# jizongFox/Contrast-You

Hardware: AMD Instinct MI355X
Metric: 2D slices/sec on ACDC U-Net+InfoNCE step (higher is better)
Workload: dtype bf16; 1 GPU; C2: ACDC SemiSupervisedEpocher + InfoNCE@Conv5 (partition), two-stage, 16 labeled + 16 unlabeled 1x224x224 per GPU, 4 classes, UNet max_channel=512, RAdam; global_batch=32, parallelism=dp1

## Files before the change

### contrast-you_amd/contrastyou/arch/unet.py

```python
from __future__ import annotations

from collections import OrderedDict
from contextlib import contextmanager
from enum import Enum
from functools import partial
from typing import Optional

import torch
from torch import Tensor, nn

from cyhip import ops
from cyhip.functions import (ChainCfg, ConvChainFn, HeadFn, begin_pass, compute_dtype_for, defer_batch_counters,
                             prepack)

from ._base import _check_params, _complete_arch_start2end
from .utils import get_bn_track, get_requires_grad

__all__ = ["UNet", "UNetFeatureMapEnum"]


def _conv3x3(cin: int, cout: int) -> nn.Conv2d:
    return nn.Conv2d(cin, cout, kernel_size=(3, 3), stride=(1, 1), padding=(1, 1), bias=False)


# ... 93 lines not shown
        self._Up_conv2 = _ConvBlock(ch("Up_conv3"), ch("Up_conv2"), momentum)

        self._Deconv_1x1 = _Head1x1(ch("Up_conv2"), num_classes, kernel_size=(1, 1), stride=(1, 1),
                                    padding=(0, 0))
        self._compute_dtype: Optional[torch.dtype] = None
        for tag, names in (("decoder", self.decoder_names), ("conv5", ("Conv5",)), ("conv4", ("Conv4",))):
            for n in names:
                for p in getattr(self, f"_{n}").parameters():
                    p.__dict__["_cy_ready_tag"] = tag
        self._Up5.ready_tag, self._Conv5.ready_tag, self._Conv4.ready_tag = "decoder", "conv5", "conv4"

    @property
    def compute_dtype(self) -> Optional[torch.dtype]:
        return self._compute_dtype

    @compute_dtype.setter
    def compute_dtype(self, dt: Optional[torch.dtype]):
        self._compute_dtype = dt
        for m in self.modules():
            if isinstance(m, (_ConvBlock, _UpConv)):
                m.compute_dtype = dt

    def forward(self, x: Tensor, until: str = None):
        if until and until not in self.layer_dimension:
            raise KeyError(f"`return_until` should be in {', '.join(self.layer_dimension.keys())},"
                           f" given {until}  ")
        ops.require_gpu(x)
        ops.note_home_stream(x.device)
        if x.dim() != 4 or x.shape[1] != self._input_dim:
            raise ValueError(f"expected [N,{self._input_dim},H,W], got {tuple(x.shape)}")
        if x.shape[2] % 16 or x.shape[3] % 16:
            raise ValueError("spatial dims must be multiples of 16 (four 2x2 poolings)")
        begin_pass()
        prepack(self._packed_conv_weights(), compute_dtype_for(x, self._compute_dtype))
        with defer_batch_counters(x.device):
            return self._forward(x, until)

    def _packed_conv_weights(self):
        ws = []
        for m in self.modules():
            if isinstance(m, _ConvBlock):
                ws += [m.conv[3].weight] if m._first else [m.conv[0].weight, m.conv[3].weight]
            elif isinstance(m, _UpConv):
                ws.append(m.up[1].weight)
        return [w for w in ws if w.is_cuda and w.dtype == torch.float32 and w.is_contiguous()]

    def _forward(self, x: Tensor, until: Optional[str]):
        e1 = self._Conv1(x, pool_out=until != "Conv1")
        if until == "Conv1":
            return e1
        e2 = self._Conv2(self._Conv1.take_pooled(), pool_out=until != "Conv2")
        if until == "Conv2":
            return e2
        e3 = self._Conv3(self._Conv2.take_pooled(), pool_out=until != "Conv3")
        if until == "Conv3":
            return e3
        e4 = self._Conv4(self._Conv3.take_pooled(), pool_out=until != "Conv4")
        if until == "Conv4":
            return e4
        e5 = self._Conv5(self._Conv4.take_pooled())
        if until == "Conv5":
            return e5

        d5 = self._Up_conv5(e4, self._Up5(e5))
        if until == "Up_conv5":
            return d5
        d4 = self._Up_conv4(e3, self._Up4(d5))
# ... 81 lines not shown
```

### contrast-you_amd/csrc/cy_conv3x3.hip

```cpp
#include "cy_conv_plane.h"
#include "cy_conv_stream.h"
#include "cy_conv_flow.h"
#include "cy_conv_tile.h"

#include <cstdlib>

namespace {

template <typename T, typename TO, int TH, int TW, int BN, int WGM, int WGN, int PITCHB, bool ALLT>
struct ConvCfg {
  static constexpr int EPC = ElemTr<T>::EPC;
  static constexpr int KC = PITCHB / (int)sizeof(T);
  static constexpr int CPP = PITCHB / 16;
  static constexpr int KS = KC / 16;
  static constexpr int HW2 = TW + 2;
  static constexpr int ZSLOT = TH + 2;
  static constexpr int A_BYTES = (TH + 3) * HW2 * PITCHB;
  static constexpr int B_BYTES = BN * PITCHB;
  static constexpr int MT = TH * TW / 32;
  static constexpr int M_REP = MT / WGM;
  static constexpr int N_REP = BN / (32 * WGN);
  static constexpr int BREG = (BN * CPP + 255) / 256;
  static constexpr int TAB_BYTES = (3 * TH + 4) * 4;
  static constexpr int EPI_BYTES = 4 * 32 * 36 * 4 + WGM * 2 * BN * 4;
  static constexpr int NBUF = ALLT ? 9 : 2;
  static constexpr int MAIN_BYTES = A_BYTES + NBUF * B_BYTES;
  static constexpr int SMEM = (MAIN_BYTES > EPI_BYTES ? MAIN_BYTES : EPI_BYTES) + TAB_BYTES + 16;
  static_assert(WGM * WGN == 4, "4 waves");
  static_assert((TH * TW) % 32 == 0 && MT % WGM == 0, "tile/wave split");
  static_assert(BN % (32 * WGN) == 0, "cout/wave split");
  static_assert(256 % CPP == 0, "chunk ownership");
};

template <typename T, typename TO, int TH, int TW, int BN, int WGM, int WGN, int PITCHB, bool ALLT>
__global__ void __launch_bounds__(256, 2)
// ... 521 lines not shown
  TileChoice tile = choose_tile(NH, d->W, Cout);
  if (plane) tile.th = kPlaneTH, tile.tw = kPlaneTW;
  const int tiles = cy_cdiv(NH, tile.th) * cy_cdiv(d->W, tile.tw);
  if (plane) {
    tile.bn = Cout >= 128 ? 128 : (Cout > 32 ? 64 : 32);
    constexpr int bn64_below = 300;
    if (Cout == 128 && tiles < bn64_below) tile.bn = 64;
  }
  const int blocks = tiles * cy_cdiv(Cout, tile.bn);
  const int kc = (tile.bn <= 64 ? 64 : 128) / (d->in_dtype == CY_F32 ? 4 : 2);
  const int ncc = cy_cdiv(Cin, kc);
  int Z = 1;
  if (blocks < 192 && ncc >= 2 && Cout % 8 == 0) {
    Z = cy_cdiv(384, blocks);
    if (Z > ncc) Z = ncc;
    if (Z > 8) Z = 8;
  }
  bool one_per_cu = false;
  if (plane && tile.bn == 128 && ncc >= 2) {
    int z1 = blocks >= 256 ? 1 : 256 / blocks;
    if (z1 > ncc / 2) z1 = ncc / 2;
    if (z1 < 1) z1 = 1;
    if (blocks * z1 >= 192 && blocks * z1 <= 288 && Cout % 8 == 0) one_per_cu = true, Z = z1;
  }
  return make_plan(d, plane ? CY_CONV_KERNEL_PLANE : CY_CONV_KERNEL_IGEMM, tile, Z, tiles, one_per_cu);
}

ConvPlan plan_conv(const cy_conv_desc* d) {
  ConvPlan p;
  if (plan_stream(d, &p) || plan_flow(d, &p)) return p;
  return plan_tiled(d);
}

template <typename TO>
int launch_finish(const ConvArgs& a, const ConvPlan& p, hipStream_t st) {
  const int G = a.Cout / 8;
  const int gpp = G < 256 ? G : 256;
  const int rows = 256 / gpp;
  const size_t smem = (size_t)2 * rows * gpp * 8 * sizeof(float);
  hipLaunchKernelGGL(conv_splitk_finish_kernel<TO>, dim3(p.finish_blocks), dim3(256), smem, st, a.ws,
                     p.ksplit, (long)a.NH * a.W, a.Cout, (TO*)a.out, a.ldo, (TO*)a.out2, a.ldo2,
                     a.split_c, a.stats, a.sacc, a.sR);
  CY_CHECK_LAUNCH();
  return CY_OK;
}

template <typename T>
int dispatch_conv(const ConvArgs& a, const ConvPlan& p, hipStream_t st) {
  if (p.kernel == CY_CONV_KERNEL_STREAM) {
    if constexpr (sizeof(T) == 2) return dispatch_conv_stream<T>(a, st);
    return CY_ERR_DTYPE;
  }
  if (p.kernel == CY_CONV_KERNEL_FLOW) {
    if constexpr (sizeof(T) == 2) return dispatch_conv_flow<T>(a, p.tile.th, p.tile.bn, p.tile.tw, st);
    return CY_ERR_DTYPE;
  }
  if (p.kernel == CY_CONV_KERNEL_PLANE) {
    if (p.tile.bn == 128)
      return p.one_per_cu ? launch_conv_plane<T, kPlaneTH, 128, 2, 2, 128, false, true>(a, st)
                          : launch_conv_plane<T, kPlaneTH, 128, 2, 2, 128, false, false>(a, st);
    if (p.tile.bn == 64) return launch_conv_plane<T, kPlaneTH, 64, 4, 1, 64, true>(a, st);
    return launch_conv_plane<T, kPlaneTH, 32, 4, 1, 64, true>(a, st);
  }
  const TileChoice c = p.tile;
#define CY_CONV_CASE(TH_, TW_, BN_, WGM_, WGN_, P_, ALLT_) \
  return launch_conv<T, T, TH_, TW_, BN_, WGM_, WGN_, P_, ALLT_>(a, st)
// ... 589 lines not shown
  a.ksplit = p.ksplit;
  a.ws = (float*)ws;
  if (p.ksplit > 1 && (!ws || ws_bytes < p.ws_bytes)) return CY_ERR_WORKSPACE;
  hipStream_t st = (hipStream_t)stream;
  if (dz) {
    if (!dgrad_dz_plan_ok(d, p, dz->c0, dz->C)) return CY_ERR_SHAPE;
    a.dz_y = dz->y, a.dz_coef = dz->coef, a.dz_acc = (unsigned long long*)dz->acc->acc, a.dz_R = dz->acc->R;
    a.dz_ld = dz->C, a.dz_c0 = dz->c0, a.dz_C = dz->C;
  }
  if (bwd) {
    if (!dgrad_bn_plan_ok(d, p)) return CY_ERR_SHAPE;
    a.ysrc = bwd->y, a.bytes_y = a.bytes1;
    a.dy_out = bwd->dy, a.bytes_dy = a.bytes1;
    a.bfold.acc = (const unsigned long long*)bwd->acc->acc, a.bfold.R = bwd->acc->R, a.bfold.C = d->C1;
    a.bfold.coef = bwd->coef, a.bfold.inv_count = 1.0 / bwd->count, a.bfold.batch_stats = bwd->batch_stats;
    a.bfold.accumulate = bwd->accumulate, a.bfold.dgamma = bwd->dgamma, a.bfold.dbeta = bwd->dbeta;
  }
  if (in_fold) {
    if ((p.kernel == CY_CONV_KERNEL_FLOW || p.kernel == CY_CONV_KERNEL_STREAM) && cy_switches().bn_fold_in_kernel) {
      a.fold = bn_fold_from_abi(in_fold);
    } else {
      rc = cy_bn_fold_coef(in_fold, stream);
      if (rc != CY_OK) return rc;
      a.scale = in_fold->coef, a.shift = in_fold->coef + in_fold->C;
    }
  }
  rc = d->in_dtype == CY_BF16 ? dispatch_conv<bf16>(a, p, st)
       : d->in_dtype == CY_F16 ? dispatch_conv<f16>(a, p, st) : dispatch_conv<float>(a, p, st);
  if (rc != CY_OK || p.ksplit == 1) return rc;
  return d->in_dtype == CY_BF16 ? launch_finish<bf16>(a, p, st)
         : d->in_dtype == CY_F16 ? launch_finish<f16>(a, p, st) : launch_finish<float>(a, p, st);
}

int cy_debug_conv_stamps(unsigned long long* dev_buf) {
  g_conv_stamp_buf = dev_buf;
  return CY_OK;
}

int cy_conv3x3_first_num_partials(int N, int H, int W, int Cout) {
  if (Cout % 8 || Cout > 64 || 256 % (Cout / 8)) return CY_ERR_SHAPE;
  const int b = first_conv_blocks((long)N * H * W, Cout, W);
  return b < 0 ? CY_ERR_SHAPE : b;
}

static int first_fwd_impl(const float* x, const float* w, void* out, float* stats, unsigned long long* sacc, int sR, int N,
                          int Cin, int H, int W, int Cout, int out_dtype, void* stream);

int cy_conv3x3_first_fwd(const float* x, const float* w, void* out, float* stats, int N, int Cin,
                         int H, int W, int Cout, int out_dtype, void* stream) {
  return first_fwd_impl(x, w, out, stats, nullptr, 0, N, Cin, H, W, Cout, out_dtype, stream);
}

int cy_conv3x3_first_fwd_acc(const float* x, const float* w, void* out, const cy_bn_acc* out_acc, int N, int Cin,
                             int H, int W, int Cout, int out_dtype, void* stream) {
  if (!out_acc || !out_acc->acc || out_acc->C != Cout || out_acc->R < 1 || (out_acc->R & (out_acc->R - 1))) return CY_ERR_ARG;
  return first_fwd_impl(x, w, out, nullptr, (unsigned long long*)out_acc->acc, out_acc->R, N, Cin, H, W, Cout, out_dtype, stream);
}

static int first_fwd_impl(const float* x, const float* w, void* out, float* stats, unsigned long long* sacc, int sR, int N,
                          int Cin, int H, int W, int Cout, int out_dtype, void* stream) {
  if (!x || !w || !out) return CY_ERR_ARG;
  if (Cin < 1 || Cin > 4) return CY_ERR_SHAPE;
  if ((long)N * H * W >= (1L << 31)) return CY_ERR_SHAPE;
  const int np = cy_conv3x3_first_num_partials(N, H, W, Cout);
  if (np < 0) return np;
  hipStream_t st = (hipStream_t)stream;
// ... 36 lines not shown
```

### contrast-you_amd/csrc/cy_switches.h

```cpp
#pragma once
#include <cstdlib>

namespace cy_env {
static inline int as_int(const char* name, int dflt) {
  const char* e = getenv(name);
  return e ? atoi(e) : dflt;
}
static inline bool unless_0(const char* name) {
  const char* e = getenv(name);
  return !(e && e[0] == '0');
}
}

struct CySwitches {
  bool conv_plane = cy_env::unless_0("CY_CONV_PLANE");
  int stream = cy_env::as_int("CY_STREAM", 1);
  int flow = cy_env::as_int("CY_FLOW", 1);
  int flow_cfg = cy_env::as_int("CY_FLOW_CFG", 0);
  int plane_xcd = cy_env::as_int("CY_PLANE_XCD", 1);
  int dgrad_bn_all = cy_env::as_int("CY_DGRAD_BN_ALL", 0);
  int bn_fold_in_kernel = cy_env::as_int("CY_BN_FOLD_IN_KERNEL", 1);
  int first_mfma = cy_env::as_int("CY_FIRST_MFMA", 1);
  bool first_wgrad_mfma = cy_env::unless_0("CY_FIRST_WGRAD_MFMA");
  bool wgrad_spec = cy_env::unless_0("CY_WGRAD_SPEC");
  bool wgrad_dma = cy_env::unless_0("CY_WGRAD_DMA");
  bool wgrad_blk = cy_env::unless_0("CY_WGRAD_BLK");
};

__attribute__((visibility("hidden"))) inline const CySwitches& cy_switches() {
  static const CySwitches s{};
  return s;
}
```

### contrast-you_amd/cyhip/functions.py

```python
from __future__ import annotations

import contextlib
import os
from typing import List, Optional

import torch
from torch import Tensor, nn

from . import ops

_weights_epoch = 0


_nbt_pending: Optional[list] = None


_run_pending: Optional[list] = None


class defer_batch_counters:

    def __init__(self, device=None):
        self._device = device

# ... 14 lines not shown
            ops.bn_running_update(running)
            if pending:
                with ops.ordered("bn_batch_counters"):
                    torch._foreach_add_(pending, 1)
        return False


RAW_TAP = None


def bump_weights_epoch() -> None:
    global _weights_epoch
    _weights_epoch += 1


def packed_weights(w: Tensor, dtype: torch.dtype):
    tag = (w._version, _weights_epoch, w.data_ptr(), torch.cuda.is_current_stream_capturing())
    cache = w.__dict__.get("_cy_pack")
    if cache is None:
        cache = w.__dict__["_cy_pack"] = {}
    hit = cache.get(dtype)
    cur = torch.cuda.current_stream(w.device)
    if hit is not None and hit[0] == tag:
        if hit[4] != cur and hit[5] == ops._capture_id(cur):
            cur.wait_event(hit[3])
        return hit[1], hit[2]
    wf, wd = ops.pack_weights(w, dtype, want_dgrad=True)
    ev = torch.cuda.Event()
    ev.record(cur)
    cache[dtype] = (tag, wf, wd, ev, cur, ops._capture_id(cur))
    return wf, wd


def prepack(weights, dtype: torch.dtype) -> None:
    if not weights:
        return
    w0 = weights[0]
    cap = torch.cuda.is_current_stream_capturing()
    hit = w0.__dict__.get("_cy_pack", {}).get(dtype)
    if hit is not None and hit[0] == (w0._version, _weights_epoch, w0.data_ptr(), cap):
        return
    cur = torch.cuda.current_stream(w0.device)
    packs = ops.pack_weights_batched([w.detach() for w in weights], dtype)
    ev = torch.cuda.Event()
    ev.record(cur)
    capid = ops._capture_id(cur)
    for w, (wf, wd) in zip(weights, packs):
        w.__dict__.setdefault("_cy_pack", {})[dtype] = ((w._version, _weights_epoch, w.data_ptr(), cap),
                                                        wf, wd, ev, cur, capid)


PAIR_WGRAD = os.environ.get("CY_PAIR_WGRAD", "1") != "0"
_parked = {}
_keepalive = []
_pass_serial = 0
_step_first_pass = None


def begin_pass() -> int:
    global _pass_serial, _step_first_pass
    _pass_serial += 1
    if _step_first_pass is None and torch.is_grad_enabled():
        _step_first_pass = _pass_serial
        if ops.marks_wanted and torch.cuda.is_available():
            ops.begin_step_marks(torch.cuda.current_device())
    return _pass_serial


class side_pass:

    def __enter__(self):
        global _step_first_pass
        self._outer, _step_first_pass = _step_first_pass, None
        return self

    def __exit__(self, *exc):
        global _step_first_pass
        _step_first_pass = self._outer
        return False


class _Parked:
# ... 105 lines not shown
        if self.fold is not None and pool_out:
            return ops.bn_relu_apply_pool_fold(self.y, self.fold)
        if self.fold is not None:
            return ops.bn_relu_apply_fold(self.y, self.fold), None
        if pool_out:
            return ops.bn_relu_apply_pool(self.y, self.scale, self.shift)
        return ops.bn_relu_apply(self.y, self.scale, self.shift), None

    def tail(self):
        return self.y, self.coef, self.acc


def _acc_backward(evals: List[_BnEval]) -> bool:
    return ops.BN_ACC and all(e.y.shape[1] <= 1024 for e in evals)



def _cast_inputs(cfg: ChainCfg, x1: Tensor, x2: Optional[Tensor], dt: torch.dtype):
    if cfg.first:
        return x1, x2
    x1 = ops.to_nhwc(x1 if x1.dtype == dt else x1.to(dt))
    if x2 is not None:
        x2 = ops.to_nhwc(x2 if x2.dtype == dt else x2.to(dt))
    return x1, x2


def _conv_fwd(cfg: ChainCfg, w: Tensor, dt: torch.dtype, src1: Tensor, src2: Optional[Tensor], prev: Optional[_BnEval],
              flags, needs_grad: bool):
    use_batch, _, on_acc = flags
    if prev is None and cfg.first:
        return ops.conv_first_fwd(src1, w, dt, want_stats=use_batch, stats_acc=on_acc)
    note_forward_use(w, needs_grad)
    wf, _ = packed_weights(w, dt)
    if prev is None:
        return ops.conv3x3_fwd(src1, src2, wf, w.shape[0], mode=cfg.mode, want_stats=use_batch, stats_acc=on_acc)
    return ops.conv3x3_fwd(prev.y, None, wf, w.shape[0], want_stats=use_batch, stats_acc=on_acc, **prev.prologue())


def _bn_eval(bn: nn.BatchNorm2d, g: Tensor, b: Tensor, y: Tensor, part, flags, run_items: list) -> _BnEval:
    use_batch, update, on_acc = flags
    count = y.shape[0] * y.shape[2] * y.shape[3]
    mom = bn.momentum if bn.momentum is not None else 0.1
    if on_acc:
        fold = ops.BnState(part, g.detach(), b.detach(), count, bn.eps, y.device)
        coef = fold.coef
        if update:
            run_items.append((coef, bn.running_mean, bn.running_var, mom))
    else:
        fold = None
        coef = ops.bn_finalize_block(part, count, g.detach(), b.detach(), bn.running_mean, bn.running_var, mom, bn.eps,
                                     use_batch, update, y.shape[1], y.device)
    if update and bn.num_batches_tracked is not None:
        if _nbt_pending is not None:
            _nbt_pending.append(bn.num_batches_tracked)
        else:
            bn.num_batches_tracked.add_(1)
    return _BnEval(y, coef, fold, use_batch)


def _running_update(run_items: list) -> None:
    if not run_items:
        return
    if _run_pending is not None:
        _run_pending.extend(run_items)
    else:
        ops.bn_running_update(run_items)
# ... 1312 lines not shown
```

### contrast-you_amd/cyhip/ops.py

```python
from __future__ import annotations

import contextlib
import os
import ctypes as C
from typing import Optional, Tuple

import torch
from torch import Tensor

from . import _lib
from ._lib import CY_BF16, CY_F16, CY_F32, CY_SRC_DIRECT, CY_SRC_POOL2, CY_SRC_UP2, ConvDesc

_DT = {torch.float32: CY_F32, torch.bfloat16: CY_BF16, torch.float16: CY_F16}
HALF_TYPES = (torch.bfloat16, torch.float16)

PROFILE = None


class TimingEvent:

    __slots__ = ("_h",)

    def __init__(self):
        h = C.c_void_p()
# ... 157 lines not shown


_pack_sets = {}


def pack_weights_batched(weights, dtype: torch.dtype):
    require_gpu(*weights)
    for w in weights:
        if w.dtype != torch.float32 or not w.is_contiguous():
            raise ValueError("pack_weights_batched wants contiguous f32 weights")
    if len(weights) > 64:
        raise ValueError("at most 64 layers per batched pack")
    key = (dtype, tuple(w.data_ptr() for w in weights), tuple(tuple(w.shape) for w in weights))
    ps = _pack_sets.get(key)
    if ps is None:
        if len(_pack_sets) > 8:
            _pack_sets.clear()
        ps = _pack_sets[key] = _PackSet(weights, dtype)
    dev = weights[0].device
    af = torch.empty(ps.size_f, dtype=dtype, device=dev)
    ad = torch.empty(ps.size_d, dtype=dtype, device=dev)
    _lib.call("cy_conv3x3_pack_weights_batched", ps.table.data_ptr(), ps.n, ps.total, af.data_ptr(),
              ad.data_ptr(), dtype_code(dtype), _stream())
    out = []
    for (of, nf), (od, nd) in ps.views:
        out.append((af[of:of + nf], ad[od:od + nd]))
    return out


_desc_cache = {}


class _Plan:
    __slots__ = ("d", "ref", "npart", "fwd_ws", "wgrad_ws", "pair_ws", "stat_wgs", "dgrad_bn")

    def __init__(self, d: ConvDesc):
        self.d, self.ref = d, C.byref(d)
        self.npart = self.fwd_ws = self.wgrad_ws = self.stat_wgs = self.dgrad_bn = None
        self.pair_ws = {}


def _desc(N, H, W, C1, C2, Cout, mode, prologue, dt, ld1, ld2, ldo, split_c=0, ldo2=0) -> _Plan:
    key = (N, H, W, C1, C2, Cout, mode, prologue, dt, ld1, ld2, ldo, split_c, ldo2)
    p = _desc_cache.get(key)
    if p is None:
        d = ConvDesc()
        d.N, d.H, d.W, d.C1, d.C2, d.Cout = N, H, W, C1, C2, Cout
        d.mode1, d.prologue, d.in_dtype, d.out_dtype = mode, prologue, dt, dt
        d.ld1, d.ld2, d.ldo, d.split_c, d.ldo2 = ld1, ld2, ldo, split_c, ldo2
        p = _desc_cache[key] = _Plan(d)
    return p


def _query(struct, name: str, *args, skip=()) -> dict:
    s = struct()
    _lib.call(name, *args, C.byref(s))
    return {f: getattr(s, f) for f, _ in s._fields_ if f not in skip}


KERNEL_NAMES = {_lib.CY_CONV_KERNEL_IGEMM: "conv3x3_igemm_kernel", _lib.CY_CONV_KERNEL_PLANE: "conv3x3_plane_kernel",
                _lib.CY_CONV_KERNEL_STREAM: "conv3x3_stream_kernel", _lib.CY_CONV_KERNEL_FLOW: "conv3x3_flow_kernel"}


def conv3x3_plan(N, H, W, C1, C2, Cout, dtype: torch.dtype, mode: int = 0, prologue: bool = False,
                 split: Optional[int] = None) -> dict:
    if split:
        d = _desc(N, H, W, C1, C2, Cout, mode, 1 if prologue else 0, dtype_code(dtype), C1, C2, split, split, Cout - split)
    else:
        d = _desc(N, H, W, C1, C2, Cout, mode, 1 if prologue else 0, dtype_code(dtype), C1, C2, Cout)
    out = _query(_lib.ConvPlan, "cy_conv3x3_plan", d.ref)
    out["kernel"] = KERNEL_NAMES[out["kernel"]]
# ... 40 lines not shown
    stats = acc = None
    if want_stats and stats_acc:
        if d.stat_wgs is None:
            d.stat_wgs = _lib.call("cy_conv3x3_stat_workgroups", d.ref)
        acc = bn_acc_new(Cout, d.stat_wgs, dev)
    elif want_stats:
        if d.npart is None:
            d.npart = _lib.call("cy_conv3x3_num_partials", d.ref)
        stats = _f32(d.npart * 2 * Cout, dev).view(d.npart, 2, Cout)
    if d.fwd_ws is None:
        d.fwd_ws = _lib.load().cy_conv3x3_fwd_ws_bytes(d.ref)
    nbytes = d.fwd_ws
    ws = _ws(nbytes, dev) if nbytes else None
    ev = _prof_begin()
    if fold is not None or acc is not None:
        _lib.call("cy_conv3x3_fwd_bn", d.ref, src1.data_ptr(), _ptr(src2), None if fold is None else fold.ref,
                  _ptr(scale), _ptr(shift), wf.data_ptr(), out.data_ptr(), _ptr(out2), None,
                  None if acc is None else acc.ref, _ptr(ws), nbytes, _stream())
        stats = acc
        if fold is not None:
            fold.done = True
    else:
        _lib.call("cy_conv3x3_fwd", d.ref, src1.data_ptr(), _ptr(src2), _ptr(scale), _ptr(shift),
                  wf.data_ptr(), out.data_ptr(), _ptr(out2), _ptr(stats), _ptr(ws), nbytes, _stream())
    if ev is not None:
        esz = src1.element_size()
        nb = esz * (src1.numel() + (0 if src2 is None else src2.numel()) + N * H * W * Cout + 9 * (C1 + C2) * Cout)
        _prof_end(ev, "conv3x3_fwd_dgrad", 2.0 * N * H * W * 9 * (C1 + C2) * Cout, float(nb))
    if split:
        return (out, out2), None
    return out, stats



ASYNC_WGRAD = os.environ.get("CY_ASYNC_WGRAD", "1") != "0"
CAPTURING = False
_side_streams = {}
_side_pending = set()


def side_stream(device, role: str = "wgrad") -> "torch.cuda.Stream":
    idx = torch.device(device).index
    if idx is None:
        idx = torch.cuda.current_device()
    st = _side_streams.get((idx, role))
    if st is None:
        st = _side_streams[(idx, role)] = torch.cuda.Stream(device=idx, priority=-1 if role == "comm" else 0)
    return st


def note_side_work(stream) -> None:
    global _multi_stream_live
    _multi_stream_live = True
    _side_pending.add(stream)


class on_side_stream:

    def __init__(self, *reads: Optional[Tensor]):
        self.reads = [t for t in reads if t is not None]

    def __enter__(self):
        dev = self.reads[0].device
        self.side = side_stream(dev)
        self.side.wait_stream(torch.cuda.current_stream(dev))
        self.ctx = torch.cuda.stream(self.side)
# ... 2492 lines not shown
```

### include/contrastyou_hip.h

```cpp
#ifndef CONTRASTYOU_HIP_H
#define CONTRASTYOU_HIP_H

#include <stddef.h>
#include <stdint.h>

#ifdef __cplusplus
extern "C" {
#endif

#define CY_OK 0
#define CY_ERR_ARG (-1)
#define CY_ERR_SHAPE (-2)
#define CY_ERR_DTYPE (-3)
#define CY_ERR_LAUNCH (-4)
#define CY_ERR_WORKSPACE (-5)

#define CY_F32 0
#define CY_BF16 1
#define CY_F16 2

#define CY_SRC_DIRECT 0
#define CY_SRC_POOL2 1
#define CY_SRC_UP2 2

// ... 158 lines not shown
int cy_maxpool2_bwd_bn_acc(const void* x, const void* dpool, const void* add, int ld_add, void* dx, const void* y,
                           const float* coef, const cy_bn_acc* acc, int N, int H, int W, int C, int dtype,
                           void* stream);
int cy_upsample2_bwd_bn_workgroups(int N, int H, int W, int C);
int cy_upsample2_bwd_bn_acc(const void* dup, int ld_dup, void* dx, const void* y, const float* coef,
                            const cy_bn_acc* acc, int N, int H, int W, int C, int dtype, void* stream);
int cy_bn_relu_bwd_apply_fold(const void* da, int ld_da, const void* y, const float* coef, const cy_bn_acc* acc,
                              double count, int batch_stats, float* dgamma, float* dbeta, int accumulate, void* dy,
                              long npix, int C, int dtype, void* stream);

typedef struct cy_bn_bwd_in {
  const void* y;
  const float* coef;
  const cy_bn_acc* acc;
  double count;
  int32_t batch_stats, accumulate;
  float* dgamma;
  float* dbeta;
  void* dy;
} cy_bn_bwd_in;
int cy_conv3x3_dgrad_bn_ok(const cy_conv_desc* d);
int cy_conv3x3_dgrad_bn(const cy_conv_desc* d, const void* dA, const cy_bn_bwd_in* bn, const void* w_packed, void* out,
                        void* out2, void* ws, size_t ws_bytes, void* stream);

typedef struct cy_bn_dz_out {
  const void* y;
  const float* coef;
  const cy_bn_acc* acc;
  int32_t c0, C;
} cy_bn_dz_out;
int cy_conv3x3_dgrad_dz_ok(const cy_conv_desc* d, int c0, int C);
int cy_conv3x3_dgrad_dz(const cy_conv_desc* d, const void* dy, const void* w_packed, void* out, void* out2,
                        const cy_bn_dz_out* dz, void* ws, size_t ws_bytes, void* stream);

int cy_conv3x3_first_num_partials(int N, int H, int W, int Cout);
int cy_conv3x3_first_fwd(const float* x, const float* w, void* out, float* stats, int N, int Cin,
                         int H, int W, int Cout, int out_dtype, void* stream);
size_t cy_conv3x3_first_wgrad_ws_bytes(int N, int Cin, int H, int W, int Cout);
int cy_conv3x3_first_wgrad(const float* x, const void* dy, float* dw, int accumulate, int N, int Cin,
                           int H, int W, int Cout, int dy_dtype, void* ws, size_t ws_bytes,
                           void* stream);

int cy_bn_finalize(const float* partials, int num_partials, int C, double count,
                   const float* gamma, const float* beta, float* running_mean,
                   float* running_var, float momentum, float eps, int use_batch_stats,
                   int update_running, float* scale, float* shift, float* mean, float* invstd,
                   void* stream);

int cy_bn_relu_apply(const void* y, const float* scale, const float* shift, void* out,
                     long npix, int C, int y_dtype, int out_dtype, void* stream);

int cy_bn_relu_apply_pool(const void* y, const float* scale, const float* shift, void* out, void* pooled,
                          int N, int H, int W, int C, int y_dtype, int out_dtype, void* stream);

int cy_bn_bwd_num_partials(long npix, int C);
int cy_bn_relu_bwd_reduce(const void* da, int ld_da, const void* y, const float* scale,
                          const float* shift, const float* mean, const float* invstd,
                          float* partials, long npix, int C, int dtype, void* stream);
int cy_bn_bwd_finalize(const float* partials, int num_partials, int C, const float* scale,
                       const float* mean, const float* invstd, double count, int batch_stats,
                       float* dgamma, float* dbeta, int accumulate, float* coef, void* stream);
int cy_bn_relu_bwd_apply(const void* da, int ld_da, const void* y, const float* scale,
                         const float* shift, const float* coef, void* dy, long npix, int C,
                         int dtype, void* stream);

int cy_maxpool2_bwd(const void* x, const void* dpool, const void* add, int ld_add, void* dx, int N,
// ... 562 lines not shown
```

Before: 5570 slices/s.

## Compute upsample-then-conv3x3 forward as four 2x2 phase convolutions at low resolution

Adds a phase-decomposed forward kernel for the nearest-upsample-by-2 followed by 3x3 conv layers. The 3x3 weights are pre-summed into four 2x2 phase kernels, so the GEMM runs on the low-resolution input with 4 taps instead of 9 on the upsampled input, which cuts MACs by more than half and avoids materialising the upsampled operand. The kernel interleaves the four phase outputs into the full-resolution NHWC result and accumulates BN stats. It also adds a separate weight-pack kernel with per-weight caching. The cost is extra packing work each time the weights change, and a new code path limited to bf16/f16 layers with BN batch stats.

```diff
diff --git a/contrast-you_amd/contrastyou/arch/unet.py b/contrast-you_amd/contrastyou/arch/unet.py
--- a/contrast-you_amd/contrastyou/arch/unet.py
+++ b/contrast-you_amd/contrastyou/arch/unet.py
@@ -149,7 +149,9 @@
         if x.shape[2] % 16 or x.shape[3] % 16:
             raise ValueError("spatial dims must be multiples of 16 (four 2x2 poolings)")
         begin_pass()
-        prepack(self._packed_conv_weights(), compute_dtype_for(x, self._compute_dtype))
+        packed = self._packed_conv_weights()
+        up2 = [m.up[1].weight for m in self.modules() if isinstance(m, _UpConv)]
+        prepack(packed, compute_dtype_for(x, self._compute_dtype), up2=[w for w in up2 if any(w is p for p in packed)])
         with defer_batch_counters(x.device):
             return self._forward(x, until)
 
diff --git a/contrast-you_amd/csrc/cy_conv3x3.hip b/contrast-you_amd/csrc/cy_conv3x3.hip
--- a/contrast-you_amd/csrc/cy_conv3x3.hip
+++ b/contrast-you_amd/csrc/cy_conv3x3.hip
@@ -1,6 +1,7 @@
 #include "cy_conv_plane.h"
 #include "cy_conv_stream.h"
 #include "cy_conv_flow.h"
+#include "cy_conv_up2.h"
 #include "cy_conv_tile.h"
 
 #include <cstdlib>
@@ -588,6 +589,29 @@
   return plan_tiled(d);
 }
 
+struct Up2Plan {
+  bool ok;
+  int th, bn, tw, tiles, workgroups;
+};
+Up2Plan plan_up2_fwd(const cy_conv_desc* d, bool acc_stats) {
+  Up2Plan p = {false, 0, 0, 0, 0, 0};
+  if (!cy_switches().up2_phase || d->mode1 != CY_SRC_UP2 || d->in_dtype == CY_F32 || !acc_stats) return p;
+  if (d->prologue || d->C2 || d->split_c > 0 || (d->H & 1) || (d->W & 1)) return p;
+  if (d->C1 % 16 || d->Cout % 64) return p;
+  if (!below_2gib(d, kSrc1 | kOut)) return p;
+  cy_conv_desc v = *d;
+  v.H = d->H / 2, v.W = d->W / 2, v.Cout = 4 * d->Cout, v.mode1 = CY_SRC_DIRECT, v.ldo = 4 * d->Cout;
+  const FlowChoice fc = flow_choice(&v);
+  if (!fc.ok) return p;
+  const FlowPick k = flow_auto_rule(&v, fc, true);
+  p.th = k.th, p.bn = k.bn, p.tw = fc.tw;
+  if (d->Cout % p.bn) p.bn = 64;
+  p.tiles = cy_cdiv((long)v.N * v.H, p.th) * (v.W / p.tw);
+  p.workgroups = p.tiles * (v.Cout / p.bn);
+  p.ok = true;
+  return p;
+}
+
 template <typename TO>
 int launch_finish(const ConvArgs& a, const ConvPlan& p, hipStream_t st) {
   const int G = a.Cout / 8;
@@ -1243,6 +1267,59 @@
          : d->in_dtype == CY_F16 ? launch_finish<f16>(a, p, st) : launch_finish<float>(a, p, st);
 }
 
+long long cy_conv3x3_up2_packed_elems(int Cout, int Cin, int dtype) {
+  if (Cout <= 0 || Cin <= 0 || (dtype != CY_BF16 && dtype != CY_F16)) return 0;
+  return up2_image_elems(Cout, Cin);
+}
+
+int cy_conv3x3_up2_pack_weights(const void* items, int n_items, long long total, void* arena, int dtype, void* stream) {
+  if (!items || n_items <= 0 || n_items > 64 || total <= 0 || total > (0x7fffffffLL << 6) || !arena) return CY_ERR_ARG;
+  hipStream_t st = (hipStream_t)stream;
+  const dim3 grid((unsigned)((4 * total + 255) / 256));
+  const cy_pack_item* tab = (const cy_pack_item*)items;
+  if (dtype == CY_BF16)
+    hipLaunchKernelGGL(up2_pack_kernel<bf16>, grid, dim3(256), 0, st, tab, n_items, total, (bf16*)arena);
+  else if (dtype == CY_F16)
+    hipLaunchKernelGGL(up2_pack_kernel<f16>, grid, dim3(256), 0, st, tab, n_items, total, (f16*)arena);
+  else
+    return CY_ERR_DTYPE;
+  CY_CHECK_LAUNCH();
+  return CY_OK;
+}
+
+int cy_conv3x3_up2_plan(const cy_conv_desc* d, int acc_stats, cy_conv_plan* plan) {
+  const int rc = conv_check(d);
+  if (rc != CY_OK) return rc;
+  if (!plan) return CY_ERR_ARG;
+  const Up2Plan p = plan_up2_fwd(d, acc_stats != 0);
+  if (!p.ok) return CY_ERR_SHAPE;
+  plan->kernel = CY_CONV_KERNEL_UP2;
+  plan->th = p.th, plan->tw = p.tw, plan->bn = p.bn;
+  plan->ksplit = 1, plan->one_per_cu = 0;
+  plan->partials = 4 * p.tiles;
+  plan->workgroups = p.workgroups;
+  return CY_OK;
+}
+
+int cy_conv3x3_up2_fwd(const cy_conv_desc* d, const void* src1, const void* w_phase, void* out, const cy_bn_acc* out_acc,
+                       void* stream) {
+  const int rc = conv_check(d);
+  if (rc != CY_OK) return rc;
+  if (!src1 || !w_phase || !out || !out_acc || !out_acc->acc) return CY_ERR_ARG;
+  if (out_acc->C != d->Cout || out_acc->R < 1 || (out_acc->R & (out_acc->R - 1))) return CY_ERR_ARG;
+  const Up2Plan p = plan_up2_fwd(d, true);
+  if (!p.ok) return CY_ERR_SHAPE;
+  Up2Args a = {};
+  a.src = src1, a.wimg = w_phase, a.out = out;
+  a.sacc = (unsigned long long*)out_acc->acc, a.sR = out_acc->R;
+  a.H = d->H / 2, a.W = d->W / 2, a.NH = d->N * a.H;
+  a.Cin = d->C1, a.Cout = d->Cout, a.ld1 = d->ld1, a.ldo = d->ldo;
+  a.bytes_src = (((long)a.NH * a.W - 1) * d->ld1 + d->C1) * 2;
+  a.bytes_w = up2_image_elems(d->Cout, d->C1) * 2;
+  hipStream_t st = (hipStream_t)stream;
+  return d->in_dtype == CY_BF16 ? dispatch_up2_fwd<bf16>(a, p.th, p.bn, p.tw, st) : dispatch_up2_fwd<f16>(a, p.th, p.bn, p.tw, st);
+}
+
 int cy_debug_conv_stamps(unsigned long long* dev_buf) {
   g_conv_stamp_buf = dev_buf;
   return CY_OK;
diff --git a/contrast-you_amd/csrc/cy_conv_up2.h b/contrast-you_amd/csrc/cy_conv_up2.h
--- /dev/null
+++ b/contrast-you_amd/csrc/cy_conv_up2.h
@@ -0,0 +1,387 @@
+#pragma once
+#include "cy_conv_flow.h"
+
+namespace {
+
+struct Up2Args {
+  const void* src;
+  const void* wimg;
+  long long bytes_src, bytes_w;
+  void* out;
+  unsigned long long* sacc;
+  int sR;
+  int H, W, NH;
+  int Cin, Cout, ld1, ldo;
+  int tiles_w, xcd_remap;
+};
+
+__host__ __device__ inline long up2_elem_index(int row, int k, int tap, int nchunk) {
+  return ((((long)(row >> 6) * nchunk + (k >> 4)) * 4 + tap) * 2 + ((k >> 3) & 1)) * 512 + (row & 63) * 8 + (k & 7);
+}
+
+inline long up2_image_elems(int Cout, int Cin) {
+  if (Cout % 64 || Cin % 16) return 0;
+  return 16L * Cout * Cin;
+}
+
+template <typename T>
+__global__ void __launch_bounds__(256)
+    up2_pack_kernel(const cy_pack_item* __restrict__ items, int n, long long total, T* __restrict__ arena) {
+  const long long tidx = (long long)blockIdx.x * 256 + threadIdx.x;
+  const long long id = tidx >> 2;
+  const int jp = (int)(tidx & 3);
+  if (id >= total) return;
+  int lo = 0, hi = n - 1;
+  while (lo < hi) {
+    const int mid = (lo + hi + 1) >> 1;
+    if (items[mid].first <= id) lo = mid; else hi = mid - 1;
+  }
+  const float* w = items[lo].w;
+  const int Cout = items[lo].Cout, Cin = items[lo].Cin;
+  const long long e = id - items[lo].first;
+  const int row = (int)(e & 63), plane = (int)((e >> 6) & 1), tap = (int)((e >> 7) & 3);
+  const int nchunk = Cin / 16;
+  const int chunk = (int)((e >> 9) % nchunk), rblk = (int)((e >> 9) / nchunk);
+  const int vrow = rblk * 64 + row;
+  const int phase = vrow / Cout, co = vrow - phase * Cout;
+  const int pa = phase >> 1, pb = phase & 1, ty = tap >> 1, tx = tap & 1;
+  const int ky0 = pa ? (ty ? 2 : 0) : (ty ? 1 : 0), ky1 = pa ? (ty ? 2 : 1) : (ty ? 2 : 0);
+  const int kx0 = pb ? (tx ? 2 : 0) : (tx ? 1 : 0), kx1 = pb ? (tx ? 2 : 1) : (tx ? 2 : 0);
+  const int ci0 = chunk * 16 + plane * 8 + 2 * jp;
+  T v[2];
+#pragma unroll
+  for (int j = 0; j < 2; ++j) {
+    const float* wp = w + ((size_t)co * Cin + ci0 + j) * 9;
+    float s = 0.f;
+    for (int ky = ky0; ky <= ky1; ++ky)
+      for (int kx = kx0; kx <= kx1; ++kx) s += wp[ky * 3 + kx];
+    v[j] = from_f32<T>(s);
+  }
+  *reinterpret_cast<unsigned*>(arena + items[lo].off_f + e * 8 + 2 * jp) =
+      (unsigned)__builtin_bit_cast(unsigned short, v[0]) | ((unsigned)__builtin_bit_cast(unsigned short, v[1]) << 16);
+}
+
+template <typename T, int TH, int BN, int WGM, int WGN, bool W16>
+__global__ void __launch_bounds__(64 * WGM * WGN, 2)
+    up2_phase_fwd_kernel(const Up2Args a) {
+#if defined(__HIP_DEVICE_COMPILE__)
+  using C = FlowCfg<T, TH, BN, WGM, WGN, W16>;
+  using M = Mma<T>;
+  constexpr int EPC = C::EPC, KC = C::KC, HP = C::HP, TW = C::TW, NW = C::NW;
+  constexpr int M_REP = C::M_REP, N_REP = C::N_REP, NAI = C::NAI;
+  constexpr int APLB = C::APLB, BPLB = C::BPLB;
+  constexpr int NBITEMS = 4 * C::CPP * (BN / 64);
+  constexpr int NBI = (NBITEMS + NW - 1) / NW;
+  constexpr unsigned OOB = 0x80000000u;
+  static_assert(4 * C::CPP * BPLB <= C::B_BYTES, "four taps fit the flow kernel's weight region");
+
+  extern __shared__ __attribute__((aligned(16))) unsigned char smem[];
+  int* s_row = reinterpret_cast<int*>(smem + 2 * C::STAGE + C::COEF_BYTES);
+  int* s_flag = s_row + (TH + 2);
+
+  const int tid = threadIdx.x;
+  const int lane = tid & 63;
+  const int wave = __builtin_amdgcn_readfirstlane(tid >> 6);
+  const int wm = wave / WGN, wn = wave % WGN;
+  const int r = lane & 31, h = lane >> 5;
+  int prow, pcol;
+  if constexpr (W16) {
+    const int grp = (r >= 4 && r < 12) || (r >= 16 && r < 20) || r >= 28;
+    prow = grp;
+    pcol = grp ? (r < 12 ? r - 4 : (r < 20 ? r - 8 : r - 16)) : (r < 4 ? r : (r < 16 ? r - 8 : r - 12));
+  } else {
+    prow = r >> 4;
+    pcol = r & 15;
+  }
+
+  const int nbk = 4 * a.Cout / BN;
+  int id = blockIdx.x;
+  if (a.xcd_remap) {
+    const int nt = gridDim.x, x = id & 7, i = id >> 3, q = nt >> 3, rr = nt & 7;
+    id = (x < rr ? x * (q + 1) : rr * (q + 1) + (x - rr) * q) + i;
+  }
+  const int tile = id / nbk, nblk = id - tile * nbk;
+  const int ct = tile % a.tiles_w;
+  const int rt = tile / a.tiles_w;
+  const int R0 = rt * TH, w0 = ct * TW;
+  const int phase = (nblk * BN) / a.Cout;
+  const int n0 = nblk * BN - phase * a.Cout;
+  const int pa = phase >> 1, pb = phase & 1;
+  const int ncc = a.Cin / KC;
+
+  auto make_rsrc = [&](const void* p, long long bytes) {
+    const unsigned long long b = (unsigned long long)p;
+    const unsigned lo = __builtin_amdgcn_readfirstlane((unsigned)b), hi = __builtin_amdgcn_readfirstlane((unsigned)(b >> 32));
+    return __builtin_amdgcn_make_buffer_rsrc((void*)(((unsigned long long)hi << 32) | lo), (short)0, (int)bytes, 0x00020000);
+  };
+  const __amdgpu_buffer_rsrc_t rs1 = make_rsrc(a.src, a.bytes_src);
+  const __amdgpu_buffer_rsrc_t rsw = make_rsrc(a.wimg, a.bytes_w);
+
+  const unsigned wlane = (unsigned)lane * 16u;
+  const unsigned wblk = (unsigned)(nblk * (BN / 64)) * (unsigned)ncc * 8192u;
+  auto b_dma = [&](int cc, auto I, int st) {
+    constexpr int i = decltype(I)::value;
+    const int j = wave + NW * i;
+    if (j >= NBITEMS) return;
+    const int tp = j / (BN / 64), half = j % (BN / 64);
+    const unsigned soff = wblk + ((unsigned)half * (unsigned)ncc + (unsigned)cc) * 8192u + (unsigned)tp * 1024u;
+    auto* dst = (__attribute__((address_space(3))) void*)(smem + st + C::A_BYTES + tp * BPLB + half * 1024);
+    __builtin_amdgcn_raw_ptr_buffer_load_lds(rsw, dst, 16, wlane, soff, 0, 0);
+  };
+  plane_static_for<0, NBI>([&](auto I) { b_dma(0, I, 0); });
+
+  for (int idx = tid; idx < 2 * C::CPP * 20; idx += C::NTHR) {
+    const int pl = idx / 20, z = idx % 20;
+    st16(smem + (pl >> 1) * C::STAGE + (pl & 1) * APLB + (C::ZB - 1 + z) * 16, u32x4{0u, 0u, 0u, 0u});
+  }
+  if (tid < TH + 2) {
+    const int R = R0 - 1 + tid;
+    s_row[tid] = (R >= 0 && R < a.NH) ? R * a.W : -1;
+  }
+  if (tid < TH) {
+    const int R = R0 + tid;
+    int f = 3;
+    if (R < a.NH) {
+      const int hh = R % a.H;
+      f = (hh == 0 ? 1 : 0) | (hh == a.H - 1 ? 2 : 0);
+    }
+    s_flag[tid] = f;
+  }
+  asm volatile("s_waitcnt lgkmcnt(0)\n\ts_barrier" ::: "memory");
+
+  const int apl = wave & 1;
+  unsigned poff[NAI];
+#pragma unroll
+  for (int i = 0; i < NAI; ++i) {
+    const int lin = ((wave >> 1) + (NW / 2) * i) * 64 + lane;
+    const int hr = lin / HP, hc = lin - hr * HP;
+    const int w = w0 - 1 + hc;
+    poff[i] = OOB;
+    if (lin < C::NPOS && w >= 0 && w < a.W) {
+      const int r1 = s_row[hr];
+      if (r1 >= 0) poff[i] = ((unsigned)(r1 + w) * (unsigned)a.ld1 + (unsigned)(apl * EPC)) * (unsigned)sizeof(T);
+    }
+  }
+  auto a_dma = [&](int cc, auto I, int st) {
+    constexpr int i = decltype(I)::value;
+    const int g = (wave >> 1) + (NW / 2) * i;
+    if (g >= C::NGA) return;
+    const unsigned soff = (unsigned)(cc * KC * (int)sizeof(T));
+    auto* dst = (__attribute__((address_space(3))) void*)(smem + st + apl * APLB + 16 + g * 1024);
+    if (g * 64 + 64 <= C::NPOS || lane < C::NPOS - g * 64)
+      __builtin_amdgcn_raw_ptr_buffer_load_lds(rs1, dst, 16, poff[i], soff, 0, 0);
+  };
+
+  int arow[M_REP][2];
+#pragma unroll
+  for (int m = 0; m < M_REP; ++m) {
+    const int ty = 2 * (wm * M_REP + m) + prow;
+    const int mid = ((ty + 1) * HP + pcol + (C::W16 ? 1 : 0)) * 16 + h * APLB;
+    const int zer = (C::ZB + pcol) * 16 + h * APLB;
+    const int fl = s_flag[ty];
+    arow[m][0] = pa ? mid : ((fl & 1) ? zer : mid - HP * 16);
+    arow[m][1] = pa ? ((fl & 2) ? zer : mid + HP * 16) : mid;
+  }
+  const int acol0 = pb * 16, acol1 = (pb + 1) * 16;
+  int bbase[N_REP];
+#pragma unroll
+  for (int n = 0; n < N_REP; ++n) bbase[n] = C::A_BYTES + ((wn * N_REP + n) * 32 + r) * 16 + h * BPLB;
+
+  f32x16 acc[M_REP][N_REP];
+#pragma unroll
+  for (int m = 0; m < M_REP; ++m)
+#pragma unroll
+    for (int n = 0; n < N_REP; ++n)
+#pragma unroll
+      for (int i = 0; i < 16; ++i) acc[m][n][i] = 0.f;
+
+  auto frag = [&](const unsigned char* p) {
+    typename M::Frag f;
+    f.v = *reinterpret_cast<const decltype(f.v)*>(p);
+    return f;
+  };
+
+  plane_static_for<0, NAI>([&](auto I) { a_dma(0, I, 0); });
+
+  typename M::Frag fa[2][M_REP], fb[2][N_REP];
+  auto load_tap = [&](int st, auto SET, auto TAP) {
+    constexpr int set = decltype(SET)::value, t = decltype(TAP)::value;
+    const unsigned char* sb = smem + st;
+    const int co = (t & 1) ? acol1 : acol0;
+#pragma unroll
+    for (int n = 0; n < N_REP; ++n) fb[set][n] = frag(sb + bbase[n] + t * 2 * BPLB);
+#pragma unroll
+    for (int m = 0; m < M_REP; ++m) fa[set][m] = frag(sb + arow[m][t >> 1] + co);
+  };
+  auto mma_set = [&](auto SET) {
+    constexpr int set = decltype(SET)::value;
+    __builtin_amdgcn_sched_barrier(0);
+    __builtin_amdgcn_s_setprio(1);
+#pragma unroll
+    for (int m = 0; m < M_REP; ++m)
+#pragma unroll
+      for (int n = 0; n < N_REP; ++n) M::mma(fb[set][n], fa[set][m], acc[m][n]);
+    __builtin_amdgcn_s_setprio(0);
+    __builtin_amdgcn_sched_barrier(0);
+  };
+  auto open_chunk = [&]() {
+    asm volatile("s_waitcnt vmcnt(0)" ::: "memory");
+    asm volatile("s_waitcnt lgkmcnt(0)\n\ts_barrier" ::: "memory");
+  };
+  int st_cur = 0, st_nxt = C::STAGE;
+  open_chunk();
+  load_tap(st_cur, TapC<0>{}, TapC<0>{});
+  for (int cc = 0; cc < ncc; ++cc) {
+    const bool more = cc + 1 < ncc;
+    plane_static_for<0, 3>([&](auto TAP) {
+      constexpr int t = decltype(TAP)::value;
+      load_tap(st_cur, TapC<(t + 1) & 1>{}, TapC<t + 1>{});
+      mma_set(TapC<t & 1>{});
+      if (more) {
+        plane_static_for<0, 3>([&](auto K) {
+          constexpr int i = t + 3 * decltype(K)::value;
+          if constexpr (i < NBI) b_dma(cc + 1, TapC<(i < NBI ? i : 0)>{}, st_nxt);
+          if constexpr (i < NAI) a_dma(cc + 1, TapC<(i < NAI ? i : 0)>{}, st_nxt);
+        });
+      }
+    });
+    if (more) {
+      open_chunk();
+      load_tap(st_nxt, TapC<0>{}, TapC<0>{});
+    }
+    mma_set(TapC<1>{});
+    const int sw = st_cur;
+    st_cur = st_nxt;
+    st_nxt = sw;
+  }
+  __syncthreads();
+
+  auto position = [&](int m, int& R, int& w) -> bool {
+    R = R0 + 2 * (wm * M_REP + m) + prow;
+    if constexpr (C::W16) {
+      w = w0 + pcol;
+      return R < a.NH && w < a.W;
+    } else {
+      w = w0 + pcol - 1;
+      return pcol >= 1 && pcol <= TW && R < a.NH && w < a.W;
+    }
+  };
+  float* sstat = reinterpret_cast<float*>(smem);
+  T* o1 = reinterpret_cast<T*>(a.out);
+  typedef float f32x2 __attribute__((ext_vector_type(2)));
+  const bool rows_full = R0 + TH <= a.NH;
+  bool col_ok;
+  {
+    int R, w;
+    (void)position(0, R, w);
+    col_ok = C::W16 ? (w < a.W) : (pcol >= 1 && pcol <= TW && w < a.W);
+  }
+  auto unpack2 = [&](unsigned wd) {
+    if constexpr (__is_same(T, bf16)) {
+      return f32x2{__uint_as_float(wd << 16), __uint_as_float(wd & 0xffff0000u)};
+    } else {
+      return f32x2{(float)__builtin_bit_cast(f16, (unsigned short)(wd & 0xffffu)),
+                   (float)__builtin_bit_cast(f16, (unsigned short)(wd >> 16))};
+    }
+  };
+  auto epilogue = [&](auto MASKED_) {
+    constexpr bool MASKED = decltype(MASKED_)::value != 0;
+#pragma unroll
+    for (int n = 0; n < N_REP; ++n) {
+      u32x2 packed[M_REP][4];
+#pragma unroll
+      for (int m = 0; m < M_REP; ++m)
+#pragma unroll
+        for (int g = 0; g < 4; ++g) {
+          T pk[4];
+#pragma unroll
+          for (int j = 0; j < 4; ++j) pk[j] = from_f32<T>(acc[m][n][4 * g + j]);
+          packed[m][g] = __builtin_bit_cast(u32x2, *reinterpret_cast<const s16x4*>(pk));
+        }
+      __builtin_amdgcn_sched_barrier(0);
+      f32x2 p1[8], p2[8];
+#pragma unroll
+      for (int i = 0; i < 8; ++i) p1[i] = p2[i] = f32x2{0.f, 0.f};
+#pragma unroll
+      for (int m = 0; m < M_REP; ++m) {
+        int R, w;
+        const bool ok = position(m, R, w);
+        const size_t gp = ((size_t)(2 * R + pa) * (size_t)(2 * a.W) + (size_t)(2 * w + pb));
+#pragma unroll
+        for (int g = 0; g < 4; ++g) {
+#pragma unroll
+          for (int k = 0; k < 2; ++k) {
+            f32x2 q = unpack2(packed[m][g][k]);
+            if constexpr (MASKED) {
+              if (!ok) q = f32x2{0.f, 0.f};
+            }
+            p1[2 * g + k] += q;
+            p2[2 * g + k] += q * q;
+          }
+        }
+#pragma unroll
+        for (int g = 0; g < 4; g += 2) {
+          u32x2 lo = packed[m][g], hi = packed[m][g + 1];
+          frag_pair_swap(lo, hi);
+          const int co = n0 + (wn * N_REP + n) * 32 + 8 * g + 8 * h;
+          if (ok) *reinterpret_cast<u32x4*>(o1 + gp * a.ldo + co) = u32x4{lo[0], lo[1], hi[0], hi[1]};
+        }
+        __builtin_amdgcn_sched_barrier(0);
+      }
+      float s1v[16], s2v[16];
+#pragma unroll
+      for (int i = 0; i < 8; ++i) {
+        const bool keep = col_ok || MASKED;
+        s1v[2 * i] = keep ? p1[i][0] : 0.f;
+        s1v[2 * i + 1] = keep ? p1[i][1] : 0.f;
+        s2v[2 * i] = keep ? p2[i][0] : 0.f;
+        s2v[2 * i + 1] = keep ? p2[i][1] : 0.f;
+      }
+      frag_stats_reduce(s1v, s2v, lane);
+      if ((lane & 1) == 0) {
+        const int reg = frag_stats_reg(lane);
+        const int col = (wn * N_REP + n) * 32 + frag_channel(reg, h);
+        sstat[(wm * 2 + 0) * BN + col] = s1v[0];
+        sstat[(wm * 2 + 1) * BN + col] = s2v[0];
+      }
+    }
+  };
+  if (rows_full) epilogue(TapC<0>{});
+  else epilogue(TapC<1>{});
+  if (a.sacc != nullptr) {
+    __syncthreads();
+    if (tid < BN) {
+      float t1, t2;
+      conv_stats_total<BN, WGM>(sstat, tid, t1, t2);
+      const int rep = (tile * 4 + phase) & (a.sR - 1);
+      bn_acc_add(a.sacc, a.sR, a.Cout, rep, 0, n0 + tid, t1);
+      bn_acc_add(a.sacc, a.sR, a.Cout, rep, 1, n0 + tid, t2);
+    }
+  }
+#endif
+}
+
+template <typename T, int TH, int BN, int WGM, int WGN, bool W16>
+int launch_up2_fwd(Up2Args a, hipStream_t st) {
+  using C = FlowCfg<T, TH, BN, WGM, WGN, W16>;
+  constexpr auto kern = up2_phase_fwd_kernel<T, TH, BN, WGM, WGN, W16>;
+  if (!cy_lds_limit_once<kern>(C::SMEM)) return CY_ERR_LAUNCH;
+  if (a.W % C::TW != 0 || a.Cout % BN != 0 || a.Cin % 16 != 0) return CY_ERR_SHAPE;
+  a.tiles_w = a.W / C::TW;
+  a.xcd_remap = cy_switches().plane_xcd;
+  dim3 grid(cy_cdiv(a.NH, TH) * a.tiles_w * (4 * a.Cout / BN), 1, 1);
+  hipLaunchKernelGGL(kern, grid, dim3(C::NTHR), C::SMEM, st, a);
+  CY_CHECK_LAUNCH();
+  return CY_OK;
+}
+
+template <typename T>
+int dispatch_up2_fwd(const Up2Args& a, int th, int bn, int tw, hipStream_t st) {
+  return flow_with_tiling(th, bn, (int)CY_ERR_SHAPE, [&](auto t) {
+    using X = decltype(t);
+    if (tw == 16) return launch_up2_fwd<T, X::TH, X::BN, X::WGM, X::WGN, true>(a, st);
+    return launch_up2_fwd<T, X::TH, X::BN, X::WGM, X::WGN, false>(a, st);
+  });
+}
+
+}
diff --git a/contrast-you_amd/csrc/cy_switches.h b/contrast-you_amd/csrc/cy_switches.h
--- a/contrast-you_amd/csrc/cy_switches.h
+++ b/contrast-you_amd/csrc/cy_switches.h
@@ -18,6 +18,7 @@
   int flow = cy_env::as_int("CY_FLOW", 1);
   int flow_cfg = cy_env::as_int("CY_FLOW_CFG", 0);
   int plane_xcd = cy_env::as_int("CY_PLANE_XCD", 1);
+  bool up2_phase = cy_env::unless_0("CY_UP2_PHASE");
   int dgrad_bn_all = cy_env::as_int("CY_DGRAD_BN_ALL", 0);
   int bn_fold_in_kernel = cy_env::as_int("CY_BN_FOLD_IN_KERNEL", 1);
   int first_mfma = cy_env::as_int("CY_FIRST_MFMA", 1);
diff --git a/contrast-you_amd/cyhip/functions.py b/contrast-you_amd/cyhip/functions.py
--- a/contrast-you_amd/cyhip/functions.py
+++ b/contrast-you_amd/cyhip/functions.py
@@ -70,7 +70,41 @@
     return wf, wd
 
 
-def prepack(weights, dtype: torch.dtype) -> None:
+def packed_up2(w: Tensor, dtype: torch.dtype) -> Tensor:
+    tag = (w._version, _weights_epoch, w.data_ptr(), torch.cuda.is_current_stream_capturing())
+    cache = w.__dict__.setdefault("_cy_pack_up2", {})
+    hit = cache.get(dtype)
+    cur = torch.cuda.current_stream(w.device)
+    if hit is not None and hit[0] == tag:
+        if hit[3] != cur and hit[4] == ops._capture_id(cur):
+            cur.wait_event(hit[2])
+        return hit[1]
+    src = w.detach()
+    if src.dtype != torch.float32 or not src.is_contiguous():
+        src = src.float().contiguous()
+    wp = ops.pack_up2_phase_batched([src], dtype)[0]
+    ev = torch.cuda.Event()
+    ev.record(cur)
+    cache[dtype] = (tag, wp, ev, cur, ops._capture_id(cur), src)
+    return wp
+
+
+def _prepack_up2(weights, dtype: torch.dtype) -> None:
+    weights = [w for w in weights if ops.up2_packed_elems(w.shape[0], w.shape[1], dtype)] if ops.UP2_PHASE else []
+    if not weights:
+        return
+    cap = torch.cuda.is_current_stream_capturing()
+    cur = torch.cuda.current_stream(weights[0].device)
+    packs = ops.pack_up2_phase_batched([w.detach() for w in weights], dtype)
+    ev = torch.cuda.Event()
+    ev.record(cur)
+    capid = ops._capture_id(cur)
+    for w, wp in zip(weights, packs):
+        w.__dict__.setdefault("_cy_pack_up2", {})[dtype] = ((w._version, _weights_epoch, w.data_ptr(), cap), wp, ev, cur,
+                                                            capid, None)
+
+
+def prepack(weights, dtype: torch.dtype, up2=()) -> None:
     if not weights:
         return
     w0 = weights[0]
@@ -86,6 +120,8 @@
     for w, (wf, wd) in zip(weights, packs):
         w.__dict__.setdefault("_cy_pack", {})[dtype] = ((w._version, _weights_epoch, w.data_ptr(), cap),
                                                         wf, wd, ev, cur, capid)
+    if dtype != torch.float32:
+        _prepack_up2(list(up2), dtype)
 
 
 PAIR_WGRAD = os.environ.get("CY_PAIR_WGRAD", "1") != "0"
@@ -257,6 +293,10 @@
         return ops.conv_first_fwd(src1, w, dt, want_stats=use_batch, stats_acc=on_acc)
     note_forward_use(w, needs_grad)
     wf, _ = packed_weights(w, dt)
+    if prev is None and cfg.mode == ops.CY_SRC_UP2 and use_batch and on_acc and ops.UP2_PHASE and dt != torch.float32 \
+            and w.dtype == torch.float32 and ops.conv3x3_up2_plan(src1.shape[0], 2 * src1.shape[2], 2 * src1.shape[3],
+                                                                  src1.shape[1], w.shape[0], dt) is not None:
+        return ops.conv3x3_up2_fwd(src1, packed_up2(w, dt), w.shape[0])
     if prev is None:
         return ops.conv3x3_fwd(src1, src2, wf, w.shape[0], mode=cfg.mode, want_stats=use_batch, stats_acc=on_acc)
     return ops.conv3x3_fwd(prev.y, None, wf, w.shape[0], want_stats=use_batch, stats_acc=on_acc, **prev.prologue())
diff --git a/contrast-you_amd/cyhip/ops.py b/contrast-you_amd/cyhip/ops.py
--- a/contrast-you_amd/cyhip/ops.py
+++ b/contrast-you_amd/cyhip/ops.py
@@ -213,11 +213,12 @@
 
 
 class _Plan:
-    __slots__ = ("d", "ref", "npart", "fwd_ws", "wgrad_ws", "pair_ws", "stat_wgs", "dgrad_bn")
+    __slots__ = ("d", "ref", "npart", "fwd_ws", "wgrad_ws", "pair_ws", "stat_wgs", "dgrad_bn", "up2")
 
     def __init__(self, d: ConvDesc):
         self.d, self.ref = d, C.byref(d)
         self.npart = self.fwd_ws = self.wgrad_ws = self.stat_wgs = self.dgrad_bn = None
+        self.up2 = False
         self.pair_ws = {}
 
 
@@ -324,6 +325,99 @@
     return out, stats
 
 
+UP2_PHASE = not os.environ.get("CY_UP2_PHASE", "1").startswith("0")
+
+
+def up2_packed_elems(Cout: int, Cin: int, dtype: torch.dtype) -> int:
+    return int(_lib.load().cy_conv3x3_up2_packed_elems(Cout, Cin, dtype_code(dtype)))
+
+
+class _Up2PackSet:
+
+    def __init__(self, weights, dtype):
+        items = (_lib.PackItem * len(weights))()
+        self.views = []
+        off = first = 0
+        for it, w in zip(items, weights):
+            Cout, Cin = w.shape[0], w.shape[1]
+            n = up2_packed_elems(Cout, Cin, dtype)
+            it.w, it.off_f, it.off_d, it.first = w.data_ptr(), off, -1, first
+            it.Cout, it.Cin = Cout, Cin
+            it.off_ff = it.off_fd = -1
+            self.views.append((off, n))
+            off += n
+            first += n // 8
+        self.n, self.size, self.total = len(weights), off, first
+        self.table = torch.frombuffer(bytearray(bytes(items)), dtype=torch.uint8).to(weights[0].device)
+
+
+_up2_pack_sets = {}
+
+
+def pack_up2_phase_batched(weights, dtype: torch.dtype):
+    require_gpu(*weights)
+    for w in weights:
+        if w.dtype != torch.float32 or not w.is_contiguous():
+            raise ValueError("pack_up2_phase_batched wants contiguous f32 weights")
+        if not up2_packed_elems(w.shape[0], w.shape[1], dtype):
+            raise ValueError(f"no phase image for a {tuple(w.shape)} weight in {dtype}")
+    if len(weights) > 64:
+        raise ValueError("at most 64 layers per batched pack")
+    key = (dtype, tuple(w.data_ptr() for w in weights), tuple(tuple(w.shape) for w in weights))
+    ps = _up2_pack_sets.get(key)
+    if ps is None:
+        if len(_up2_pack_sets) > 8:
+            _up2_pack_sets.clear()
+        ps = _up2_pack_sets[key] = _Up2PackSet(weights, dtype)
+    arena = torch.empty(ps.size, dtype=dtype, device=weights[0].device)
+    _lib.call("cy_conv3x3_up2_pack_weights", ps.table.data_ptr(), ps.n, ps.total, arena.data_ptr(), dtype_code(dtype),
+              _stream())
+    return [arena[o:o + n] for o, n in ps.views]
+
+
+def _up2_desc(N, H, W, C1, Cout, dtype: torch.dtype) -> _Plan:
+    d = _desc(N, H, W, C1, 0, Cout, CY_SRC_UP2, 0, dtype_code(dtype), C1, 0, Cout)
+    if d.up2 is False:
+        plan = _lib.ConvPlan()
+        rc = getattr(_lib.load(), "cy_conv3x3_up2_plan")(d.ref, 1, C.byref(plan))
+        if rc == _lib.CY_ERR_SHAPE:
+            d.up2 = None
+        else:
+            _lib.check(rc, "cy_conv3x3_up2_plan")
+            d.up2 = {f: getattr(plan, f) for f, _ in plan._fields_}
+    return d
+
+
+def conv3x3_up2_plan(N, H, W, C1, Cout, dtype: torch.dtype, acc_stats: bool = True) -> Optional[dict]:
+    if acc_stats:
+        return _up2_desc(N, H, W, C1, Cout, dtype).up2
+    d = _desc(N, H, W, C1, 0, Cout, CY_SRC_UP2, 0, dtype_code(dtype), C1, 0, Cout)
+    plan = _lib.ConvPlan()
+    rc = getattr(_lib.load(), "cy_conv3x3_up2_plan")(d.ref, 0, C.byref(plan))
+    if rc == _lib.CY_ERR_SHAPE:
+        return None
+    _lib.check(rc, "cy_conv3x3_up2_plan")
+    return {f: getattr(plan, f) for f, _ in plan._fields_}
+
+
+def conv3x3_up2_fwd(src1: Tensor, wp: Tensor, Cout: int, out: Optional[Tensor] = None):
+    require_gpu(src1, wp)
+    N, C1 = src1.shape[0], src1.shape[1]
+    H, W = 2 * src1.shape[2], 2 * src1.shape[3]
+    d = _up2_desc(N, H, W, C1, Cout, src1.dtype)
+    if d.up2 is None:
+        raise ValueError("the phase form does not apply to this layer (conv3x3_up2_plan)")
+    if out is None:
+        out = empty_nhwc(N, Cout, H, W, src1.dtype, src1.device)
+    acc = bn_acc_new(Cout, d.up2["partials"], src1.device)
+    ev = _prof_begin()
+    _lib.call("cy_conv3x3_up2_fwd", d.ref, src1.data_ptr(), wp.data_ptr(), out.data_ptr(), acc.ref, _stream())
+    if ev is not None:
+        nb = src1.element_size() * (src1.numel() + N * H * W * Cout + 9 * C1 * Cout)
+        _prof_end(ev, "conv3x3_fwd_dgrad", 2.0 * N * H * W * 9 * C1 * Cout, float(nb))
+    return out, acc
+
+
 
 ASYNC_WGRAD = os.environ.get("CY_ASYNC_WGRAD", "1") != "0"
 CAPTURING = False
diff --git a/include/contrastyou_hip.h b/include/contrastyou_hip.h
--- a/include/contrastyou_hip.h
+++ b/include/contrastyou_hip.h
@@ -214,6 +214,13 @@
 int cy_conv3x3_dgrad_dz_ok(const cy_conv_desc* d, int c0, int C);
 int cy_conv3x3_dgrad_dz(const cy_conv_desc* d, const void* dy, const void* w_packed, void* out, void* out2,
                         const cy_bn_dz_out* dz, void* ws, size_t ws_bytes, void* stream);
+
+#define CY_CONV_KERNEL_UP2 6
+long long cy_conv3x3_up2_packed_elems(int Cout, int Cin, int dtype);
+int cy_conv3x3_up2_pack_weights(const void* items, int n_items, long long total, void* arena, int dtype, void* stream);
+int cy_conv3x3_up2_plan(const cy_conv_desc* d, int acc_stats, cy_conv_plan* plan);
+int cy_conv3x3_up2_fwd(const cy_conv_desc* d, const void* src1, const void* w_phase, void* out, const cy_bn_acc* out_acc,
+                       void* stream);
 
 int cy_conv3x3_first_num_partials(int N, int H, int W, int Cout);
 int cy_conv3x3_first_fwd(const float* x, const float* w, void* out, float* stats, int N, int Cin,
```

Measured after the change: 5592 slices/s, median of 6. About the same (+0.4%).
